# swacisko/ALGA

Hardware: AMD Instinct MI355X
Metric: overlap_edges_per_sec (higher is better)
Workload: dtype u32; 1 GPU; cfg4_50M_150bp: 50000000 x 150 bp reads, genome 250000000, seed 11, err 0.00 -> 90621096 nodes (both strands, duplicates removed), min_overlap 82, rsoemo 116; generated on the device (alga_amd.workload.device_build) in 1.0 s; nodes=90621096, edges=92350115

## Files before the change

alga_amd/csrc/engine.hip:

```cpp
#include <hip/hip_runtime.h>

#include <algorithm>
#include <chrono>
#include <cstdio>
#include <cstdlib>
#include <cstring>
#include <new>
#include <string>
#include <thread>
#include <vector>

#include "engine_internal.h"
#include "prefsuf_shard.h"

using namespace alga;

namespace {

using Prepared = AlgaPrepared;

int prepare(alga_engine *e, const alga_nodes *nodes, const alga_prefsuf_params *p, hipStream_t s, Prepared &out) {
    if (!nodes || !p) return alga_fail(e, ALGA_ERR_INVALID_ARGUMENT, "nodes/params must not be NULL");
    if (nodes->n < 0) return alga_fail(e, ALGA_ERR_INVALID_ARGUMENT, "negative node count");
    if (nodes->n > 0 && (!nodes->words || !nodes->len)) return alga_fail(e, ALGA_ERR_INVALID_ARGUMENT, "words/len must not be NULL");
// ... 5 lines not shown
    if (p->keys_shared < 0 || p->keys_shared > 2) return alga_fail(e, ALGA_ERR_INVALID_ARGUMENT, "keys_shared must be 0, 1 or 2");
    int rc;
    if ((rc = alga_ensure(e, e->counters, (CNT_TOTAL + 2) * sizeof(unsigned long long)))) return rc;
    HIP_TRY(e, hipMemsetAsync(e->counters.p, 0, (CNT_TOTAL + 2) * sizeof(unsigned long long), s));
    NodesDev nd;
    nd.words = nodes->words; nd.len = nodes->len; nd.from = nodes->align_from; nd.to = nodes->align_to;
    nd.n = nodes->n; nd.stride = nodes->stride_words;
    unsigned long long *cnt = (unsigned long long *) e->counters.p;
    int *d_maxlen = (int *) (cnt + CNT_TOTAL);
    unsigned long long mask_asym = 0;
    int min_len = 0;
    if (p->keys_shared == 2 && e->store_n == nodes->n && e->store_words == (const void *) nodes->words && e->stat_len == (const void *) nodes->len &&
        e->stat_from == (const void *) nodes->align_from && e->stat_to == (const void *) nodes->align_to) {
        out.max_len = e->stat_max_len; out.live = e->stat_live; mask_asym = e->stat_mask_asym; min_len = e->stat_min_len;
    } else {
        launch_node_stats(nd, cnt, d_maxlen, s);
        if ((rc = alga_check_launch(e, "k_node_stats"))) return rc;
        HIP_TRY(e, hipMemcpyAsync(e->h_counters, e->counters.p, (CNT_TOTAL + 2) * sizeof(unsigned long long), hipMemcpyDeviceToHost, s));
        HIP_TRY(e, hipStreamSynchronize(s));
        out.max_len = (int) (e->h_counters[CNT_TOTAL] & 0xFFFFFFFFull);
        min_len = out.max_len > 0 ? 0x7FFFFFFF - (int) (e->h_counters[CNT_TOTAL] >> 32) : 0;
        out.live = e->h_counters[CNT_LIVE_NODES];
        mask_asym = e->h_counters[CNT_MASK_ASYM];
        e->stat_max_len = out.max_len; e->stat_min_len = min_len; e->stat_live = out.live; e->stat_mask_asym = mask_asym;
        e->stat_len = (const void *) nodes->len; e->stat_from = (const void *) nodes->align_from; e->stat_to = (const void *) nodes->align_to;
    }
    out.nd = nd;
    out.uniform_len = (out.max_len > 0 && min_len == out.max_len && !nodes->align_from) ? out.max_len : 0;
    if ((int64_t) blocks_of(out.max_len) > (int64_t) nodes->stride_words)
        return alga_fail(e, ALGA_ERR_INVALID_ARGUMENT, "stride_words is smaller than the longest read needs");
    if (out.max_len > OL_MAX_NODE_LEN) return alga_fail(e, ALGA_ERR_CAPACITY, "a node is longer than 4 194 303 nt (overlap records keep the offset in 22 bits)");
// ... 107 lines not shown
        if ((rc = cluster_alloc(e, pp))) return rc;
        if (pp.keys_shared == 2) {
            const bool store_left = e->store_n == nd.n && e->store_words == (const void *) nd.words && e->store_eq == pp.cluster_eq && e->store_buckets == cc.n_buckets;
            const bool piles_serve = pile && e->pile_kept_pure && e->store_buckets == cc.n_buckets && e->store_eq == pp.cluster_eq;
            if (!(store_left || piles_serve) || src_begin < e->store_run_begin || src_end > e->store_run_end)
                return alga_fail(e, ALGA_ERR_INVALID_ARGUMENT, "keys_shared = 2: no entry array of this node set that covers the sources is left from the previous build");
            keys_only = pile && e->pile_keys_only;
        } else {
            int32_t run_begin = 0, run_end = nd.n;
            if (pp.keys_shared == 1) {
                if (e->keyed_n != nd.n || e->keyed_words != (const void *) nd.words || src_begin < e->keyed_begin || src_end > e->keyed_end)
                    return alga_fail(e, ALGA_ERR_INVALID_ARGUMENT, "keys_shared: alga_prefsuf_keys_device has not been called on this node set for a range that covers the sources");
                run_begin = e->keyed_begin; run_end = e->keyed_end;
            } else {
                keys_only = pile && e->opt_pile_runs != 0 && !e->expect_pairwise && !e->opt_pile_check;
                launch_cluster_keys(nd, cfg, cc, 0, nd.n, (uint32_t *) e->cl_keys[0].p, need_vals ? (uint32_t *) e->cl_vals[0].p : nullptr, (uint32_t *) e->cl_meta.p, e->cl_runs.p,
                                    (uint8_t *) e->cl_nruns.p, s, !keys_only);
                if ((rc = alga_check_launch(e, "k_node_runs"))) return rc;
            }
            HIP_TRY(e, hipEventRecord(e->ev[EV_KEYS], s));
            e->keyed_n = -1;
            e->store_n = -1;
            HIP_TRY(e, launch_cluster_sort(nd, cc, (uint32_t *) e->cl_keys[0].p, (uint32_t *) e->cl_vals[0].p, (uint32_t *) e->cl_keys[1].p,
                                           (uint32_t *) e->cl_vals[1].p, e->sort_temp.p, cluster_sort_temp_bytes((uint64_t) nd.n), pp.keys_shared == 1 || !need_vals,
                                           e->ev[EV_SORT], e->opt_test_unsorted_index != 0, s, e->opt_own_sort != 0));
            const bool dir_late = pile && e->opt_pile_dir >= 1;
            e->dir_late = dir_late;
            if (!dir_late) {
                HIP_TRY(e, launch_cluster_dir(nd, cc, (const uint32_t *) e->cl_keys[1].p, e->cl_dir.p, cnt + CNT_TOTAL + 1, nullptr, s));
                HIP_TRY(e, hipEventRecord(e->ev[EV_DIR], s));
            }
            e->pile_n = -1;
            if (pile) {
                rc = e->opt_test_pile_oom ? alga_fail(e, ALGA_ERR_OUT_OF_MEMORY, "pile_alloc (option test_pile_oom)") : pile_alloc(e, (uint64_t) nd.n, cc.n_buckets, s);
                if (rc == ALGA_ERR_OUT_OF_MEMORY) {
                    (void) hipGetLastError();
                    alga_release(e->cl_pile_tab); alga_release(e->cl_pile_rec); alga_release(e->cl_pile_rec2); alga_release(e->cl_pile_succ); alga_release(e->cl_pile_own);
                    alga_release(e->cl_pile_list);
                    e->pile_epoch = 0; e->pile_n = -1;
                    e->err.clear();
                    pile = false;
                    rc = ALGA_OK;
                    if (keys_only) {
                        launch_cluster_keys(nd, cfg, cc, 0, nd.n, (uint32_t *) e->cl_keys[0].p, (uint32_t *) e->cl_vals[0].p, (uint32_t *) e->cl_meta.p, e->cl_runs.p,
                                            (uint8_t *) e->cl_nruns.p, s, true);
                        if ((rc = alga_check_launch(e, "k_node_runs"))) return rc;
                        keys_only = false;
                    }
                } else if (rc) return rc;
            }
            if (pile) {
                launch_pile_sample(nd, cc, pp.uniform_len, (const uint32_t *) e->cl_keys[1].p, (const uint32_t *) e->cl_vals[1].p, e->cl_dir.p,
                                   (unsigned long long *) e->cl_pile_cnt.p, e->opt_pile >= 2 ? e->opt_pile - 1 : 0, s, e->opt_pile_dir >= 1);
                if ((rc = alga_check_launch(e, "k_pile_build<sample>"))) return rc;
            }
            e->pile_tab_index = pile && e->opt_pile_dir >= 2 && e->opt_pile_skip_gather && !cfg.stats;
            if (dir_late) {
                HIP_TRY(e, hipEventRecord(e->ev[EV_SAMPLE], s));
                HIP_TRY(e, launch_cluster_dir(nd, cc, (const uint32_t *) e->cl_keys[1].p, e->cl_dir.p, cnt + CNT_TOTAL + 1,
                                              e->pile_tab_index ? (const unsigned long long *) e->cl_pile_cnt.p : nullptr, s));
                HIP_TRY(e, hipEventRecord(e->ev[EV_DIR], s));
            }
            HIP_TRY(e, launch_cluster_gather(nd, cc, pp.cluster_eq, (const uint32_t *) e->cl_keys[1].p, (const uint32_t *) e->cl_vals[1].p, (const uint32_t *) e->cl_meta.p,
                                             pp.uniform_len, e->cl_store.p, (pile && e->opt_pile_skip_gather) ? (const unsigned long long *) e->cl_pile_cnt.p : nullptr, s));
            HIP_TRY(e, hipEventRecord(e->ev[EV_GATHER], s));
            if (pile) {
                if (e->pile_epoch >= 511u) {
                    HIP_TRY(e, hipMemsetAsync(e->cl_pile_tab.p, 0, e->cl_pile_tab.cap, s));
                    e->pile_epoch = 0;
                }
                e->pile_epoch++;
                const bool from_consensus = e->opt_pile_runs != 0;
                launch_pile_build(nd, cfg, cc, pp.uniform_len, (const uint32_t *) e->cl_keys[1].p, (const uint32_t *) e->cl_vals[1].p, e->cl_dir.p, e->cl_pile_rec.p, e->cl_pile_rec2.p, e->cl_pile_tab.p,
                                  e->pile_epoch, e->cl_pile_succ.p, e->cl_runs.p, pp.uniform_len - cfg.Lmin + 1, (const unsigned long long *) e->cl_pile_cnt.p,
                                  from_consensus ? (uint32_t *) e->cl_pile_own.p : nullptr, (from_consensus && e->opt_pile_runs_list) ? e->cl_pile_list.p : nullptr, s,
// ... 1175 lines not shown
```

alga_amd/csrc/prefsuf_cluster.hip:

```cpp
#include <hip/hip_runtime.h>
#include <algorithm>
#include "prefsuf_common.h"
#include "prefsuf_kernels.h"
#include "prefsuf_device.h"
#include "prefsuf_cluster_device.h"

namespace alga {


template <int TKW, bool WIDE, bool RUNS>
__global__ void __launch_bounds__(TK_ROWS) k_node_runs(NodesDev nd, PrefSufCfg cfg, ClusterCfg cc, int node_begin, int node_end,
                                                        uint32_t *__restrict__ keys, uint32_t *__restrict__ vals, uint32_t *__restrict__ meta,
                                                        uint2 *__restrict__ runs, uint8_t *__restrict__ nruns, const int32_t *__restrict__ id_list, const unsigned long long *__restrict__ id_count,
                                                        const unsigned long long *__restrict__ only_if_declined ) {
    if (only_if_declined && !pile_cnt_declines(only_if_declined)) return;
    __shared__ uint32_t s[TK_ROWS][TKW];
    __shared__ uint32_t stk[RUNS ? 2 * (NR_STACK + 1) : 1][TK_ROWS];
    __shared__ uint16_t rbuf[RUNS ? CL_RMAX + 1 : 1][TK_ROWS];
    const int list_n = id_list ? (int) min((unsigned long long) (node_end - node_begin), *id_count) : 0;
    __shared__ int sid[TK_ROWS];
    for (int blk = (int) blockIdx.x; id_list ? blk * TK_ROWS < list_n : node_begin + blk * TK_ROWS < node_end; blk += (int) gridDim.x) {
    const int base = node_begin + blk * TK_ROWS;
    const int nrows = id_list ? min(TK_ROWS, list_n - blk * TK_ROWS) : min(TK_ROWS, node_end - base);
    if (blk != (int) blockIdx.x) __syncthreads();
    if (id_list) {
// ... 66 lines not shown
            const uint32_t pk = order_key0(kmer_hash(funnel(x0, x1, r) & cc.lo_mask, funnel(x1, x2, r) & cc.hi_mask), e);
            cur0 = pk < cur0 ? pk : cur0;
        }
    }
    uint32_t key = 0xFFFFFFFFu, m = act ? (((uint32_t) len << 8) | (is_src ? CL_META_FROM : 0u)) : 0u;
    if (is_tgt) {
        uint32_t pmin = cur0;
        if (pmin == 0xFFFFFFFFu) {
            for (int k = 0; k < w; k++) { uint32_t h, pk; kmer_key(row, k, true, cc, h, pk); pmin = pk < pmin ? pk : pmin; }
        }
        uint32_t h, pk;
        kmer_key(row, (int) (pmin & 255u), true, cc, h, pk);
        key = tgt_sort_key(cluster_key(h, fs), pmin & 255u, fs);
        m = (pmin & 255u) | ((uint32_t) len << 8) | (is_src ? CL_META_FROM : 0u);
    }
    if (in) { keys[i] = key; if (vals) vals[i] = (uint32_t) i; meta[i] = m; }
    }
}

template <int EQ, bool UNIFORM>
__global__ void __launch_bounds__(256) k_tgt_gather(NodesDev nd, uint64_t count ,
                                                     const uint32_t *__restrict__ keys, const uint32_t *__restrict__ vals,
                                                     const uint32_t *__restrict__ meta, uint32_t uniform_meta, int fs, uint4 *__restrict__ store,
                                                     const unsigned long long *__restrict__ pile_cnt ) {
    if (pile_cnt && pile_cnt[1] * PILE_IRREGULAR_ONE_IN <= pile_cnt[0]) return;
    for (uint64_t t = (uint64_t) blockIdx.x * blockDim.x + threadIdx.x; t < count * EQ; t += (uint64_t) gridDim.x * blockDim.x) {
    const uint64_t j = t / EQ;
    const int c = (int) (t % EQ);
    const uint32_t key = keys[j];
    const uint32_t id = vals[j];
    const uint32_t *row = nd.words + (size_t) id * nd.stride;
// ... 8 lines not shown
        if (!UNIFORM) v.w = meta[id];
        else if (key != 0xFFFFFFFFu) v.w = uniform_meta | ((key >> fs) & ((1u << CL_MBITS) - 1u));
        else v.w = (uint32_t) nd.len[id] == (uniform_meta >> 8 & 0xFFFu) ? uniform_meta : 0u;
    }
    store[j * EQ + c] = v;
    }
}

constexpr int TD_TILE = 256, TD_HALO = 96;
__global__ void __launch_bounds__(TD_TILE) k_tgt_dir(const uint32_t *__restrict__ keys, uint64_t n, int shift, uint32_t n_buckets ,
                                                     uint32_t bucket_base , uint4 *__restrict__ dir,
                                                     unsigned long long *__restrict__ bad ,
                                                     const unsigned long long *__restrict__ pile_cnt ) {
    if (pile_cnt && pile_cnt_pure(pile_cnt)) return;
    __shared__ uint32_t sb[TD_TILE + TD_HALO + 1];
    const uint64_t base = (uint64_t) blockIdx.x * TD_TILE;
    const uint32_t nb3 = n_buckets << 3;
    auto tagged = [&](uint64_t k) -> uint32_t { if (k >= n) return nb3; const uint32_t x = keys[k]; return x == 0xFFFFFFFFu ? nb3 : (x >> (shift - 3)) - (bucket_base << 3); };
    for (int k = (int) threadIdx.x; k <= TD_TILE + TD_HALO; k += TD_TILE)
        sb[k] = (base == 0 && k == 0) ? 0xFFFFFFFFu : tagged(base + (uint64_t) k - 1u);
    __syncthreads();
    const int t = (int) threadIdx.x, lane = lane_id();
    const uint64_t j = base + (uint64_t) t;
    auto put = [&](int64_t b, const uint4 &rec) { dir[b] = rec; };
    auto tally = [](unsigned long long acc, uint32_t cls) { return acc + (0x0101010101010100ull << (8u * cls)); };
    if (j >= 1 && j < n && sb[t + 1] < sb[t]) atomicOr(bad, 1ull);
    const uint32_t b = sb[t + 1] >> 3;
    const bool start = j <= n && b != (sb[t] >> 3);
    if (start && b == n_buckets) put(b, make_uint4((uint32_t) j, 0u, 0u, 0u));
    const bool real = start && b != n_buckets;
    constexpr int TD_SHORT = 4;
    const bool is_short = real && (sb[t + 1 + TD_SHORT] >> 3) != b;
    if (is_short) {
// ... 47 lines not shown
            if (past) {
                for (; k < j0 + 256u; k++) {
                    const uint32_t x = tagged(k);
                    if ((x >> 3) != bb) break;
                    acc = tally(acc, x & 7u);
                }
                if (k >= j0 + 256u && (tagged(k) >> 3) == bb) {
                    uint64_t a = k, z = n;
                    while (z - a > 1) { const uint64_t mid = a + (z - a) / 2; if ((tagged(mid) >> 3) == bb) a = mid; else z = mid; }
                    k = z;
                }
            }
            const uint32_t c = (uint32_t) (k - j0);
            put(bb, make_uint4((uint32_t) j0, c, c <= 255u ? (uint32_t) acc : 0u, c <= 255u ? (uint32_t) (acc >> 32) : 0u));
        }
    }
}

#ifndef CL_OCC
#define CL_OCC 6
#endif

struct ByIdEntries {
    const uint32_t *skeys, *sids;
    uint32_t uniform_meta;
    const unsigned long long *pile_cnt;
    BucketIndex bx;
};
__device__ __forceinline__ void by_id_pair(const ByIdEntries &by, size_t ei, uint32_t n_nodes, uint32_t &key, uint32_t &id) {
    key = by.skeys[ei];
// ... 812 lines not shown
    c->idx_shift = 32 - bits;
    *eq = e;
    return true;
}

size_t cluster_sort_temp_bytes(uint64_t n) { return sort_u32_pairs_temp_bytes(n); }

void launch_cluster_keys(const NodesDev &nd, const PrefSufCfg &cfg, const ClusterCfg &cc, int32_t node_begin, int32_t node_end, uint32_t *keys, uint32_t *vals,
                         uint32_t *meta, void *runs, uint8_t *nruns, hipStream_t s, bool with_runs, const unsigned long long *only_if_declined) {
    if (node_end <= node_begin) return;
    const uint64_t m = (uint64_t) (node_end - node_begin);
    const unsigned long long *gate = only_if_declined;
    const dim3 grid((unsigned) (gate ? std::min<uint64_t>((m + TK_ROWS - 1) / TK_ROWS, 8192) : (m + TK_ROWS - 1) / TK_ROWS)), block(TK_ROWS);
    const int32_t *nol = nullptr; const unsigned long long *noc = nullptr;
#define NR_LAUNCH(TKW, WIDE) do { if (with_runs) hipLaunchKernelGGL((k_node_runs<TKW, WIDE, true>), grid, block, 0, s, nd, cfg, cc, (int) node_begin, (int) node_end, keys, vals, meta, (uint2 *) runs, nruns, nol, noc, gate); \
                                  else hipLaunchKernelGGL((k_node_runs<TKW, WIDE, false>), grid, block, 0, s, nd, cfg, cc, (int) node_begin, (int) node_end, keys, vals, meta, (uint2 *) runs, nruns, nol, noc, gate); } while (0)
    if (blocks_of(cfg.Lcap - 1) > 13 || (cfg.Lcap - 1) - cfg.Lmin + 1 > 64) NR_LAUNCH(21, true);
    else if (blocks_of(cfg.Lcap - 1) <= 9) NR_LAUNCH(11, false);
    else NR_LAUNCH(17, false);
#undef NR_LAUNCH
}

void launch_cluster_runs_list(const NodesDev &nd, const PrefSufCfg &cfg, const ClusterCfg &cc, const int32_t *ids, const unsigned long long *count, uint32_t cap, uint32_t grid_blocks,
                              void *runs, uint8_t *nruns, hipStream_t s) {
    if (cap == 0 || nd.n <= 0) return;
    const dim3 grid(std::max<uint32_t>(1u, std::min<uint32_t>(grid_blocks, (cap + TK_ROWS - 1) / TK_ROWS))), block(TK_ROWS);
    uint32_t *nok = nullptr;
#define NR_LAUNCH(TKW, WIDE) hipLaunchKernelGGL((k_node_runs<TKW, WIDE, true>), grid, block, 0, s, nd, cfg, cc, 0, (int) cap, nok, nok, nok, (uint2 *) runs, nruns, ids, count, (const unsigned long long *) nullptr)
    if (blocks_of(cfg.Lcap - 1) > 13 || (cfg.Lcap - 1) - cfg.Lmin + 1 > 64) NR_LAUNCH(21, true);
    else if (blocks_of(cfg.Lcap - 1) <= 9) NR_LAUNCH(11, false);
    else NR_LAUNCH(17, false);
#undef NR_LAUNCH
}

__global__ void __launch_bounds__(256) k_iota(uint32_t *__restrict__ v, uint32_t n) {
    for (uint32_t i = blockIdx.x * 256u + threadIdx.x; i < n; i += gridDim.x * 256u) v[i] = i;
}

hipError_t launch_cluster_store(const NodesDev &nd, const ClusterCfg &cc, uint32_t *keys, uint32_t *vals, uint32_t *keys2, uint32_t *vals2,
                                void *sort_temp, size_t sort_temp_bytes, void *dir, bool fill_vals,
                                hipEvent_t ev_sorted, unsigned long long *bad_flag, bool test_skip_sort, hipStream_t s, bool own_sort) {
    const hipError_t err = launch_cluster_sort(nd, cc, keys, vals, keys2, vals2, sort_temp, sort_temp_bytes, fill_vals, ev_sorted, test_skip_sort, s, own_sort);
    return err != hipSuccess ? err : launch_cluster_dir(nd, cc, keys2, dir, bad_flag, nullptr, s);
}

hipError_t launch_cluster_sort(const NodesDev &nd, const ClusterCfg &cc, uint32_t *keys, uint32_t *vals, uint32_t *keys2, uint32_t *vals2, void *sort_temp, size_t sort_temp_bytes,
                               bool fill_vals, hipEvent_t ev_sorted, bool test_skip_sort, hipStream_t s, bool own_sort) {
    if (nd.n <= 0) return hipSuccess;
    const uint64_t n = (uint64_t) nd.n;
    if (fill_vals && (!own_sort || test_skip_sort)) hipLaunchKernelGGL(k_iota, dim3((unsigned) std::min<uint64_t>((n + 255) / 256, 8192)), dim3(256), 0, s, vals, (uint32_t) n);
    hipError_t err = hipSuccess;
    if (test_skip_sort) {
        err = hipMemcpyAsync(keys2, keys, n * sizeof(uint32_t), hipMemcpyDeviceToDevice, s);
        if (err == hipSuccess) err = hipMemcpyAsync(vals2, vals, n * sizeof(uint32_t), hipMemcpyDeviceToDevice, s);
    } else err = sort_u32_pairs(sort_temp, sort_temp_bytes, keys, keys2, own_sort ? (const uint32_t *) nullptr : vals, vals2, n, cc.idx_shift - 3, s, own_sort);
    if (err != hipSuccess) return err;
    if (ev_sorted) (void) hipEventRecord(ev_sorted, s);
    return hipSuccess;
// ... 1 lines not shown

constexpr int DF_UNROLL = 4;
__global__ void __launch_bounds__(256) k_dir_fill(uint4 *__restrict__ dir, uint64_t n_rec, const unsigned long long *__restrict__ pile_cnt) {
    if (pile_cnt && pile_cnt_pure(pile_cnt)) return;
    const uint4 z = make_uint4(0u, 0u, 0u, 0u);
    for (uint64_t p = (uint64_t) blockIdx.x * (256u * DF_UNROLL); p < n_rec; p += (uint64_t) gridDim.x * (256u * DF_UNROLL)) {
#pragma unroll
        for (int u = 0; u < DF_UNROLL; u++) {
            const uint64_t i = p + (uint64_t) u * 256u + threadIdx.x;
            if (i < n_rec) dir[i] = z;
        }
    }
}

hipError_t launch_cluster_dir(const NodesDev &nd, const ClusterCfg &cc, const uint32_t *keys2, void *dir, unsigned long long *bad_flag, const unsigned long long *only_if_no_pure_piles,
                              hipStream_t s) {
    if (nd.n <= 0) return hipSuccess;
    const uint64_t n = (uint64_t) nd.n, n_rec = (uint64_t) cc.n_buckets + 2;
    if (only_if_no_pure_piles)
        hipLaunchKernelGGL(k_dir_fill, dim3((unsigned) std::min<uint64_t>((n_rec + 256 * DF_UNROLL - 1) / (256 * DF_UNROLL), 1u << 17)), dim3(256), 0, s, (uint4 *) dir, n_rec,
                           only_if_no_pure_piles);
    else {
        const hipError_t err = hipMemsetAsync(dir, 0, n_rec * 16, s);
        if (err != hipSuccess) return err;
    }
    hipLaunchKernelGGL(k_tgt_dir, dim3((unsigned) ((n + 1 + TD_TILE - 1) / TD_TILE)), dim3(TD_TILE), 0, s, keys2, n, cc.idx_shift, cc.n_buckets, 0u, (uint4 *) dir, bad_flag, only_if_no_pure_piles);
    return hipGetLastError();
}

hipError_t launch_cluster_gather(const NodesDev &nd, const ClusterCfg &cc, int eq, const uint32_t *keys2, const uint32_t *vals2, const uint32_t *meta, int uniform_len,
                                 void *store, const unsigned long long *pile_cnt, hipStream_t s) {
    if (nd.n <= 0) return hipSuccess;
    const uint64_t n = (uint64_t) nd.n;
    const uint64_t pieces = n * (uint64_t) eq;
    const unsigned g = (unsigned) std::min<uint64_t>((pieces + 255) / 256, 1u << 16);
    const int fs = cc.idx_shift - CL_MBITS;
    const uint32_t um = uniform_len > 0 ? (((uint32_t) uniform_len << 8) | CL_META_FROM) : 0u;
#define TG_LAUNCH(E, U) hipLaunchKernelGGL((k_tgt_gather<E, U>), dim3(g), dim3(256), 0, s, nd, n, keys2, vals2, meta, um, fs, (uint4 *) store, pile_cnt)
#define TG_EQ(E) do { if (uniform_len > 0) TG_LAUNCH(E, true); else TG_LAUNCH(E, false); } while (0)
    if (eq == 2)      TG_EQ(2);
    else if (eq == 3) TG_EQ(3);
// ... 138 lines not shown
```

alga_amd/csrc/prefsuf_kernels.h:

```cpp
#pragma once
#include <hip/hip_runtime.h>
#include <stddef.h>
#include <stdint.h>
#include "prefsuf_common.h"

namespace alga {

struct alga_edge_dev { int32_t src, dst, offset; };

void launch_restride(const uint32_t *in, int stride_in, uint32_t *out, int stride_out, uint64_t n, hipStream_t s);
void launch_widen_len(const void *in, int elem_bytes , int32_t *out, uint64_t n, hipStream_t s);
void launch_compact_edges(const alga_edge_dev *edges, int32_t n, uint64_t n_edges, uint8_t *deg, uint32_t *dst, uint8_t *off, unsigned long long *bad, hipStream_t s);
void launch_expand_twins(const uint32_t *in, int stride_in, const int32_t *len , uint32_t *out, int stride_out, uint64_t n_pairs, hipStream_t s);
void launch_node_stats(const NodesDev &nd, unsigned long long *counters, int *max_len , hipStream_t s);

uint32_t seed_buckets_for(uint64_t live_nodes, int fill_x10);
uint32_t seed_filter_bits_for(uint64_t live_nodes);
void launch_seed_build(const NodesDev &nd, const PrefSufCfg &cfg, unsigned long long *table, uint32_t n_buckets, uint32_t *filter,
                       uint32_t filter_bits, hipStream_t s);

struct ProbeBig { int32_t *list; uint32_t list_cap; uint32_t count; void *items; uint32_t item_cap; };
int    local_item_capacity();
int    local_big_limit();
size_t probe_big_bytes(int n_cu, uint32_t count, int local, uint32_t item_cap);

void launch_probe(const NodesDev &nd, const PrefSufCfg &cfg, const unsigned long long *table, uint32_t n_buckets,
                  const uint32_t *filter, uint32_t filter_bits, int32_t src_begin, int32_t src_end, uint32_t *rec_dst, unsigned long long *rec_val, uint64_t rec_cap,
                  unsigned long long *counters, int n_cu, int local , uint32_t *deg , unsigned long long *first ,
                  const ProbeBig *big , hipStream_t s);
// ... 5 lines not shown

bool       cluster_plan(const PrefSufCfg &cfg, int max_len, uint64_t live, int bucket_log2_bias, ClusterCfg *c, int *eq);
size_t     cluster_sort_temp_bytes(uint64_t n);
void       launch_cluster_keys(const NodesDev &nd, const PrefSufCfg &cfg, const ClusterCfg &cc, int32_t node_begin, int32_t node_end, uint32_t *keys,
                               uint32_t *vals, uint32_t *meta, void *runs, uint8_t *nruns, hipStream_t s, bool with_runs = true ,
                               const unsigned long long *only_if_declined = nullptr );
void       launch_cluster_runs_list(const NodesDev &nd, const PrefSufCfg &cfg, const ClusterCfg &cc, const int32_t *ids, const unsigned long long *count, uint32_t cap,
                                    uint32_t grid_blocks, void *runs, uint8_t *nruns, hipStream_t s);
hipError_t launch_cluster_store(const NodesDev &nd, const ClusterCfg &cc, uint32_t *keys, uint32_t *vals, uint32_t *keys2 , uint32_t *vals2, void *sort_temp,
                                size_t sort_temp_bytes, void *dir, bool fill_vals, hipEvent_t ev_sorted ,
                                unsigned long long *bad_flag ,
                                bool test_skip_sort , hipStream_t s, bool own_sort = true);
hipError_t launch_cluster_sort(const NodesDev &nd, const ClusterCfg &cc, uint32_t *keys, uint32_t *vals, uint32_t *keys2, uint32_t *vals2, void *sort_temp, size_t sort_temp_bytes,
                               bool fill_vals, hipEvent_t ev_sorted, bool test_skip_sort, hipStream_t s, bool own_sort = true);
hipError_t launch_cluster_dir(const NodesDev &nd, const ClusterCfg &cc, const uint32_t *keys2, void *dir, unsigned long long *bad_flag, const unsigned long long *only_if_no_pure_piles,
                              hipStream_t s);
hipError_t launch_cluster_gather(const NodesDev &nd, const ClusterCfg &cc, int eq, const uint32_t *keys2, const uint32_t *vals2, const uint32_t *meta,
                                 int uniform_len , void *store,
                                 const unsigned long long *pile_cnt , hipStream_t s);
uint64_t   cluster_record_slack(int n_cu, uint64_t n_src);
void       launch_probe_clustered(const NodesDev &nd, const PrefSufCfg &cfg, const ClusterCfg &cc, int eq, const void *store, const void *dir,
                                  const void *runs, const uint8_t *nruns, int32_t src_begin, int32_t src_end, const int32_t *src_list, int32_t src_base, uint32_t *rec_dst, unsigned long long *rec_val, uint64_t rec_cap,
                                  unsigned long long *counters, int n_cu, uint32_t *deg, unsigned long long *first, const ProbeBig *big,
                                  const unsigned long long *list_count ,
                                  int sw , hipStream_t s,
                                  const uint32_t *skeys = nullptr, const uint32_t *sids = nullptr, int uniform_len = 0,
                                  const unsigned long long *pile_cnt = nullptr ,
                                  const void *tab = nullptr , uint32_t epoch = 0);
void       launch_probe_stream(const NodesDev &nd, const PrefSufCfg &cfg, const ClusterCfg &cc, int eq, const void *store, const void *dir,
                               const void *runs, const uint8_t *nruns, int32_t src_begin, int32_t src_end, bool by_key ,
                               unsigned long long *counters, int n_cu, uint32_t *deg, unsigned long long *first, unsigned long long *second, int32_t *defer_list,
// ... 90 lines not shown
```

alga_amd/csrc/prefsuf_kernels.hip:

```cpp
#include <hip/hip_runtime.h>
#include <algorithm>
#include "prefsuf_common.h"
#include "prefsuf_kernels.h"
#include "prefsuf_device.h"
#include "prefsuf_cluster_device.h"

namespace alga {

__global__ void __launch_bounds__(256) k_node_stats(NodesDev nd, unsigned long long *counters, int *max_len) {
    __shared__ int s_max[4], s_min[4];
    __shared__ unsigned long long s_live[4];
    int m = 0, mn = 0x7FFFFFFF;
    unsigned long long live = 0, asym = 0;
    auto one = [&](int l, int64_t i) {
        m = l > m ? l : m;
        mn = (l > 0 && l < mn) ? l : mn;
        live += l > 0;
        if (nd.to && l > 0 && !nd.to[i] && (nd.from == nullptr || nd.from[i])) asym++;
    };
    const int64_t gid = (int64_t) blockIdx.x * blockDim.x + threadIdx.x, gsz = (int64_t) gridDim.x * blockDim.x;
    int64_t done = 0;
    if ((reinterpret_cast<uintptr_t>(nd.len) & 15u) == 0) {
        const int64_t nq = (int64_t) nd.n >> 2;
        const int4 *len4 = reinterpret_cast<const int4 *>(nd.len);
        for (int64_t q = gid; q < nq; q += gsz) { const int4 l = len4[q]; one(l.x, 4 * q); one(l.y, 4 * q + 1); one(l.z, 4 * q + 2); one(l.w, 4 * q + 3); }
        done = 4 * nq;
    }
    for (int64_t i = done + gid; i < nd.n; i += gsz) one(nd.len[i], i);
#pragma unroll
    for (int o = 32; o > 0; o >>= 1) { int t = __shfl_xor(m, o); m = t > m ? t : m; t = __shfl_xor(mn, o); mn = t < mn ? t : mn; }
    live = wave_sum_u64(live);
    asym = wave_sum_u64(asym);
    const int wave = (int) (threadIdx.x >> 6);
    if (lane_id() == 0) { s_max[wave] = m; s_min[wave] = mn; s_live[wave] = live; if (asym) atomicAdd(&counters[CNT_MASK_ASYM], asym); }
    __syncthreads();
    if (threadIdx.x == 0) {
        for (int w = 1; w < 4; w++) { m = s_max[w] > m ? s_max[w] : m; mn = s_min[w] < mn ? s_min[w] : mn; live += s_live[w]; }
        if (m > 0) { atomicMax(max_len, m); atomicMax(max_len + 1, 0x7FFFFFFF - mn); }
        if (live) atomicAdd(&counters[CNT_LIVE_NODES], live);
    }
}

__device__ __forceinline__ uint32_t seed_bucket(uint64_t h, uint32_t n_buckets) { return __umulhi((uint32_t) h, n_buckets); }
__device__ __forceinline__ uint32_t seed_taglen(uint64_t h, int len) {
    return ((uint32_t) (h >> 41) << 9) | (uint32_t) (len > 511 ? 511 : len);
}

__device__ __forceinline__ uint32_t seed_filter_index(uint64_t h, uint32_t filter_mask) { return (uint32_t) (h >> 32) & filter_mask; }

__global__ void __launch_bounds__(256) k_seed_build(NodesDev nd, PrefSufCfg cfg, unsigned long long *table, uint32_t n_buckets,
                                                     uint32_t *filter, uint32_t filter_mask) {
    int i = blockIdx.x * blockDim.x + threadIdx.x;
    if (i >= nd.n) return;
    int len = nd.len[i];
// ... 920 lines not shown
            if (piled && (v[k].x == 0u || v[k].y == 0u)) a = f2[g];
            if (piled && (v[k].z == 0u || v[k].w == 0u)) b = f2[g + 1];
            s += source_degree(v[k].x, piled, a.x) + source_degree(v[k].y, piled, a.y) + source_degree(v[k].z, piled, b.x) + source_degree(v[k].w, piled, b.y);
        }
    } else {
        for (int k = 0; k < SCAN_ITEMS; k++) {
            const uint64_t i = base + (uint64_t) k * SCAN_BLOCK + threadIdx.x;
            if (i < n) { const uint32_t dg = deg[i]; s += source_degree(dg, piled, (piled && dg == 0u) ? first[i] : LOCAL_FIRST_NONE); }
        }
    }
    uint32_t tot;
    block_exclusive_scan(s, &tot, lds);
    if (threadIdx.x == 0) tile_sums[blockIdx.x] = tot;
}

__global__ void __launch_bounds__(1024) k_scan_spine_serial(uint64_t *tile_sums, uint32_t n_tiles) {
    __shared__ uint64_t lds[16];
    const int lane = lane_id(), wave = (int) (threadIdx.x >> 6);
    const uint64_t per = ((uint64_t) n_tiles + 1023u) / 1024u;
    const uint64_t beg = min((uint64_t) threadIdx.x * per, (uint64_t) n_tiles), end = min(beg + per, (uint64_t) n_tiles);
    uint64_t sum = 0;
    for (uint64_t i = beg; i < end; i++) sum += tile_sums[i];
    uint64_t inc = sum;
#pragma unroll
    for (int o = 1; o < 64; o <<= 1) {
        const uint32_t lo = (uint32_t) __shfl_up((int) (uint32_t) inc, o), hi = (uint32_t) __shfl_up((int) (uint32_t) (inc >> 32), o);
        if (lane >= o) inc += ((uint64_t) hi << 32) | lo;
    }
    if (lane == 63) lds[wave] = inc;
    __syncthreads();
    uint64_t run = inc - sum;
    for (int w = 0; w < wave; w++) run += lds[w];
    for (uint64_t i = beg; i < end; i++) { const uint64_t v = tile_sums[i]; tile_sums[i] = run; run += v; }
    if (threadIdx.x == 1023) tile_sums[n_tiles] = run;
}

__global__ void __launch_bounds__(SCAN_BLOCK) k_emit_scan_tiles(int32_t src_base, uint64_t n, const uint32_t *__restrict__ deg, const unsigned long long *__restrict__ first,
                                                                 const unsigned long long *__restrict__ second, const unsigned long long *__restrict__ pile_cnt,
                                                                 const uint64_t *__restrict__ tile_sums, uint32_t *__restrict__ out, alga_edge_dev *__restrict__ edges,
                                                                 uint32_t slot_stride) {
    __shared__ uint32_t lds[8];
    const bool piled = pile_cnt != nullptr && !pile_cnt_declines(pile_cnt);
    const int lane = lane_id(), wave = (int) (threadIdx.x >> 6);
    const uint64_t wbase = (uint64_t) blockIdx.x * SCAN_TILE + (uint64_t) wave * (64 * SCAN_ITEMS) + (uint64_t) lane;
    uint32_t d[SCAN_ITEMS];
    unsigned long long f[SCAN_ITEMS];
#pragma unroll
    for (int k = 0; k < SCAN_ITEMS; k++) { const uint64_t i = wbase + 64u * k; d[k] = i < n ? deg[i] : 0u; }
#pragma unroll
// ... 137 lines not shown
    if (n_edges == 0) return;
    hipLaunchKernelGGL(k_compact_edges, dim3((unsigned) std::min<uint64_t>((n_edges + 255) / 256, 1u << 16)), dim3(256), 0, s, edges, n, n_edges, deg, dst, off, bad);
}

void launch_expand_twins(const uint32_t *in, int stride_in, const int32_t *len, uint32_t *out, int stride_out, uint64_t n_pairs, hipStream_t s) {
    if (n_pairs == 0) return;
    hipLaunchKernelGGL(k_expand_twins, dim3((unsigned) std::min<uint64_t>((n_pairs * (uint64_t) stride_out + 255) / 256, 1u << 16)), dim3(256), 0, s, in, stride_in, len, out,
                       stride_out, n_pairs);
}

void launch_restride(const uint32_t *in, int stride_in, uint32_t *out, int stride_out, uint64_t n, hipStream_t s) {
    if (n == 0) return;
    hipLaunchKernelGGL(k_restride, dim3((unsigned) std::min<uint64_t>((n * (uint64_t) stride_out + 255) / 256, 1u << 16)), dim3(256), 0, s, in, stride_in, out, stride_out, n);
}

void launch_node_stats(const NodesDev &nd, unsigned long long *counters, int *max_len, hipStream_t s) {
    if (nd.n <= 0) return;
    unsigned g = std::min<unsigned>(grid_for((uint64_t) nd.n, 256), 1024u);
    hipLaunchKernelGGL(k_node_stats, dim3(g), dim3(256), 0, s, nd, counters, max_len);
}

uint32_t seed_buckets_for(uint64_t live, int fill_x10) {
    if (fill_x10 < 5) fill_x10 = 5;
    if (fill_x10 > 60) fill_x10 = 60;
    uint64_t nb = (live * 10 + (uint64_t) fill_x10 - 1) / (uint64_t) fill_x10;
    if (nb < 64) nb = 64;
    return (uint32_t) std::min<uint64_t>(nb, 0x7FFFFFFFull);
}

uint32_t seed_filter_bits_for(uint64_t live) {
    const uint64_t want = live * 8;
    uint64_t bits = 1ull << 16;
    while (bits < want) bits <<= 1;
    if (bits <= (1ull << 25)) return (uint32_t) bits;
// ... 201 lines not shown
```

Measured before the change: 5.485 billion edges/s.

## Retune node stats, directory, key and spine-scan kernels for grid and throughput

Several unrelated kernel-level changes. k_node_stats now uses 1024-thread blocks with unrolled int4 loads, an alignment head, a CU-sized grid, and a single block-level atomic for the asymmetry counter. k_tgt_dir becomes grid-strided and is capped to a chip-sized grid when piles may skip it. k_node_runs skips writing meta when only keys are needed and lengths are uniform. The serial spine scan is rewritten as a chunked, LDS-staged, coalesced block scan with prefetch. These target launch overhead, uncoalesced serial memory access and redundant stores, at the risk of lower parallelism in the capped grids.

After: 5.518 billion edges/s (median of 6 runs). Within noise of the previous version (+0.6%).

```diff
diff --git a/alga_amd/csrc/engine.hip b/alga_amd/csrc/engine.hip
--- a/alga_amd/csrc/engine.hip
+++ b/alga_amd/csrc/engine.hip
@@ -43,7 +43,7 @@
         e->stat_from == (const void *) nodes->align_from && e->stat_to == (const void *) nodes->align_to) {
         out.max_len = e->stat_max_len; out.live = e->stat_live; mask_asym = e->stat_mask_asym; min_len = e->stat_min_len;
     } else {
-        launch_node_stats(nd, cnt, d_maxlen, s);
+        launch_node_stats(nd, cnt, d_maxlen, e->n_cu, s);
         if ((rc = alga_check_launch(e, "k_node_stats"))) return rc;
         HIP_TRY(e, hipMemcpyAsync(e->h_counters, e->counters.p, (CNT_TOTAL + 2) * sizeof(unsigned long long), hipMemcpyDeviceToHost, s));
         HIP_TRY(e, hipStreamSynchronize(s));
@@ -181,8 +181,8 @@
                 run_begin = e->keyed_begin; run_end = e->keyed_end;
             } else {
                 keys_only = pile && e->opt_pile_runs != 0 && !e->expect_pairwise && !e->opt_pile_check;
-                launch_cluster_keys(nd, cfg, cc, 0, nd.n, (uint32_t *) e->cl_keys[0].p, need_vals ? (uint32_t *) e->cl_vals[0].p : nullptr, (uint32_t *) e->cl_meta.p, e->cl_runs.p,
-                                    (uint8_t *) e->cl_nruns.p, s, !keys_only);
+                launch_cluster_keys(nd, cfg, cc, 0, nd.n, (uint32_t *) e->cl_keys[0].p, need_vals ? (uint32_t *) e->cl_vals[0].p : nullptr,
+                                    (keys_only && pp.uniform_len > 0) ? nullptr : (uint32_t *) e->cl_meta.p, e->cl_runs.p, (uint8_t *) e->cl_nruns.p, s, !keys_only);
                 if ((rc = alga_check_launch(e, "k_node_runs"))) return rc;
             }
             HIP_TRY(e, hipEventRecord(e->ev[EV_KEYS], s));
@@ -194,7 +194,7 @@
             const bool dir_late = pile && e->opt_pile_dir >= 1;
             e->dir_late = dir_late;
             if (!dir_late) {
-                HIP_TRY(e, launch_cluster_dir(nd, cc, (const uint32_t *) e->cl_keys[1].p, e->cl_dir.p, cnt + CNT_TOTAL + 1, nullptr, s));
+                HIP_TRY(e, launch_cluster_dir(nd, cc, (const uint32_t *) e->cl_keys[1].p, e->cl_dir.p, cnt + CNT_TOTAL + 1, nullptr, e->n_cu, s));
                 HIP_TRY(e, hipEventRecord(e->ev[EV_DIR], s));
             }
             e->pile_n = -1;
@@ -225,7 +225,7 @@
             if (dir_late) {
                 HIP_TRY(e, hipEventRecord(e->ev[EV_SAMPLE], s));
                 HIP_TRY(e, launch_cluster_dir(nd, cc, (const uint32_t *) e->cl_keys[1].p, e->cl_dir.p, cnt + CNT_TOTAL + 1,
-                                              e->pile_tab_index ? (const unsigned long long *) e->cl_pile_cnt.p : nullptr, s));
+                                              e->pile_tab_index ? (const unsigned long long *) e->cl_pile_cnt.p : nullptr, e->n_cu, s));
                 HIP_TRY(e, hipEventRecord(e->ev[EV_DIR], s));
             }
             HIP_TRY(e, launch_cluster_gather(nd, cc, pp.cluster_eq, (const uint32_t *) e->cl_keys[1].p, (const uint32_t *) e->cl_vals[1].p, (const uint32_t *) e->cl_meta.p,
diff --git a/alga_amd/csrc/prefsuf_cluster.hip b/alga_amd/csrc/prefsuf_cluster.hip
--- a/alga_amd/csrc/prefsuf_cluster.hip
+++ b/alga_amd/csrc/prefsuf_cluster.hip
@@ -8,7 +8,7 @@
 namespace alga {
 
 
-template <int TKW, bool WIDE, bool RUNS>
+template <int TKW, bool WIDE, bool RUNS, bool META = true>
 __global__ void __launch_bounds__(TK_ROWS) k_node_runs(NodesDev nd, PrefSufCfg cfg, ClusterCfg cc, int node_begin, int node_end,
                                                         uint32_t *__restrict__ keys, uint32_t *__restrict__ vals, uint32_t *__restrict__ meta,
                                                         uint2 *__restrict__ runs, uint8_t *__restrict__ nruns, const int32_t *__restrict__ id_list, const unsigned long long *__restrict__ id_count,
@@ -105,7 +105,7 @@
         key = tgt_sort_key(cluster_key(h, fs), pmin & 255u, fs);
         m = (pmin & 255u) | ((uint32_t) len << 8) | (is_src ? CL_META_FROM : 0u);
     }
-    if (in) { keys[i] = key; if (vals) vals[i] = (uint32_t) i; meta[i] = m; }
+    if (in) { keys[i] = key; if (vals) vals[i] = (uint32_t) i; if (META) meta[i] = m; }
     }
 }
 
@@ -144,9 +144,12 @@
                                                      const unsigned long long *__restrict__ pile_cnt ) {
     if (pile_cnt && pile_cnt_pure(pile_cnt)) return;
     __shared__ uint32_t sb[TD_TILE + TD_HALO + 1];
-    const uint64_t base = (uint64_t) blockIdx.x * TD_TILE;
     const uint32_t nb3 = n_buckets << 3;
     auto tagged = [&](uint64_t k) -> uint32_t { if (k >= n) return nb3; const uint32_t x = keys[k]; return x == 0xFFFFFFFFu ? nb3 : (x >> (shift - 3)) - (bucket_base << 3); };
+    const uint64_t n_tiles = (n + 1 + TD_TILE - 1) / TD_TILE;
+    for (uint64_t tile = blockIdx.x; tile < n_tiles; tile += gridDim.x) {
+    const uint64_t base = tile * TD_TILE;
+    if (tile != blockIdx.x) __syncthreads();
     for (int k = (int) threadIdx.x; k <= TD_TILE + TD_HALO; k += TD_TILE)
         sb[k] = (base == 0 && k == 0) ? 0xFFFFFFFFu : tagged(base + (uint64_t) k - 1u);
     __syncthreads();
@@ -224,6 +227,7 @@
             const uint32_t c = (uint32_t) (k - j0);
             put(bb, make_uint4((uint32_t) j0, c, c <= 255u ? (uint32_t) acc : 0u, c <= 255u ? (uint32_t) (acc >> 32) : 0u));
         }
+    }
     }
 }
 
@@ -1066,7 +1070,8 @@
     const dim3 grid((unsigned) (gate ? std::min<uint64_t>((m + TK_ROWS - 1) / TK_ROWS, 8192) : (m + TK_ROWS - 1) / TK_ROWS)), block(TK_ROWS);
     const int32_t *nol = nullptr; const unsigned long long *noc = nullptr;
 #define NR_LAUNCH(TKW, WIDE) do { if (with_runs) hipLaunchKernelGGL((k_node_runs<TKW, WIDE, true>), grid, block, 0, s, nd, cfg, cc, (int) node_begin, (int) node_end, keys, vals, meta, (uint2 *) runs, nruns, nol, noc, gate); \
-                                  else hipLaunchKernelGGL((k_node_runs<TKW, WIDE, false>), grid, block, 0, s, nd, cfg, cc, (int) node_begin, (int) node_end, keys, vals, meta, (uint2 *) runs, nruns, nol, noc, gate); } while (0)
+                                  else if (meta) hipLaunchKernelGGL((k_node_runs<TKW, WIDE, false>), grid, block, 0, s, nd, cfg, cc, (int) node_begin, (int) node_end, keys, vals, meta, (uint2 *) runs, nruns, nol, noc, gate); \
+                                  else hipLaunchKernelGGL((k_node_runs<TKW, WIDE, false, false>), grid, block, 0, s, nd, cfg, cc, (int) node_begin, (int) node_end, keys, vals, meta, (uint2 *) runs, nruns, nol, noc, gate); } while (0)
     if (blocks_of(cfg.Lcap - 1) > 13 || (cfg.Lcap - 1) - cfg.Lmin + 1 > 64) NR_LAUNCH(21, true);
     else if (blocks_of(cfg.Lcap - 1) <= 9) NR_LAUNCH(11, false);
     else NR_LAUNCH(17, false);
@@ -1093,7 +1098,7 @@
                                 void *sort_temp, size_t sort_temp_bytes, void *dir, bool fill_vals,
                                 hipEvent_t ev_sorted, unsigned long long *bad_flag, bool test_skip_sort, hipStream_t s, bool own_sort) {
     const hipError_t err = launch_cluster_sort(nd, cc, keys, vals, keys2, vals2, sort_temp, sort_temp_bytes, fill_vals, ev_sorted, test_skip_sort, s, own_sort);
-    return err != hipSuccess ? err : launch_cluster_dir(nd, cc, keys2, dir, bad_flag, nullptr, s);
+    return err != hipSuccess ? err : launch_cluster_dir(nd, cc, keys2, dir, bad_flag, nullptr, 0 , s);
 }
 
 hipError_t launch_cluster_sort(const NodesDev &nd, const ClusterCfg &cc, uint32_t *keys, uint32_t *vals, uint32_t *keys2, uint32_t *vals2, void *sort_temp, size_t sort_temp_bytes,
@@ -1125,17 +1130,20 @@
 }
 
 hipError_t launch_cluster_dir(const NodesDev &nd, const ClusterCfg &cc, const uint32_t *keys2, void *dir, unsigned long long *bad_flag, const unsigned long long *only_if_no_pure_piles,
-                              hipStream_t s) {
+                              int n_cu, hipStream_t s) {
     if (nd.n <= 0) return hipSuccess;
     const uint64_t n = (uint64_t) nd.n, n_rec = (uint64_t) cc.n_buckets + 2;
+    const uint64_t chip = (uint64_t) std::max(1, n_cu) * 64u;
     if (only_if_no_pure_piles)
-        hipLaunchKernelGGL(k_dir_fill, dim3((unsigned) std::min<uint64_t>((n_rec + 256 * DF_UNROLL - 1) / (256 * DF_UNROLL), 1u << 17)), dim3(256), 0, s, (uint4 *) dir, n_rec,
+        hipLaunchKernelGGL(k_dir_fill, dim3((unsigned) std::min<uint64_t>((n_rec + 256 * DF_UNROLL - 1) / (256 * DF_UNROLL), chip)), dim3(256), 0, s, (uint4 *) dir, n_rec,
                            only_if_no_pure_piles);
     else {
         const hipError_t err = hipMemsetAsync(dir, 0, n_rec * 16, s);
         if (err != hipSuccess) return err;
     }
-    hipLaunchKernelGGL(k_tgt_dir, dim3((unsigned) ((n + 1 + TD_TILE - 1) / TD_TILE)), dim3(TD_TILE), 0, s, keys2, n, cc.idx_shift, cc.n_buckets, 0u, (uint4 *) dir, bad_flag, only_if_no_pure_piles);
+    const uint64_t tiles = (n + 1 + TD_TILE - 1) / TD_TILE;
+    hipLaunchKernelGGL(k_tgt_dir, dim3((unsigned) (only_if_no_pure_piles ? std::min<uint64_t>(tiles, chip) : tiles)), dim3(TD_TILE), 0, s, keys2, n, cc.idx_shift, cc.n_buckets, 0u, (uint4 *) dir,
+                       bad_flag, only_if_no_pure_piles);
     return hipGetLastError();
 }
 
diff --git a/alga_amd/csrc/prefsuf_kernels.h b/alga_amd/csrc/prefsuf_kernels.h
--- a/alga_amd/csrc/prefsuf_kernels.h
+++ b/alga_amd/csrc/prefsuf_kernels.h
@@ -12,7 +12,7 @@
 void launch_widen_len(const void *in, int elem_bytes , int32_t *out, uint64_t n, hipStream_t s);
 void launch_compact_edges(const alga_edge_dev *edges, int32_t n, uint64_t n_edges, uint8_t *deg, uint32_t *dst, uint8_t *off, unsigned long long *bad, hipStream_t s);
 void launch_expand_twins(const uint32_t *in, int stride_in, const int32_t *len , uint32_t *out, int stride_out, uint64_t n_pairs, hipStream_t s);
-void launch_node_stats(const NodesDev &nd, unsigned long long *counters, int *max_len , hipStream_t s);
+void launch_node_stats(const NodesDev &nd, unsigned long long *counters, int *max_len , int n_cu, hipStream_t s);
 
 uint32_t seed_buckets_for(uint64_t live_nodes, int fill_x10);
 uint32_t seed_filter_bits_for(uint64_t live_nodes);
@@ -48,7 +48,7 @@
 hipError_t launch_cluster_sort(const NodesDev &nd, const ClusterCfg &cc, uint32_t *keys, uint32_t *vals, uint32_t *keys2, uint32_t *vals2, void *sort_temp, size_t sort_temp_bytes,
                                bool fill_vals, hipEvent_t ev_sorted, bool test_skip_sort, hipStream_t s, bool own_sort = true);
 hipError_t launch_cluster_dir(const NodesDev &nd, const ClusterCfg &cc, const uint32_t *keys2, void *dir, unsigned long long *bad_flag, const unsigned long long *only_if_no_pure_piles,
-                              hipStream_t s);
+                              int n_cu , hipStream_t s);
 hipError_t launch_cluster_gather(const NodesDev &nd, const ClusterCfg &cc, int eq, const uint32_t *keys2, const uint32_t *vals2, const uint32_t *meta,
                                  int uniform_len , void *store,
                                  const unsigned long long *pile_cnt , hipStream_t s);
diff --git a/alga_amd/csrc/prefsuf_kernels.hip b/alga_amd/csrc/prefsuf_kernels.hip
--- a/alga_amd/csrc/prefsuf_kernels.hip
+++ b/alga_amd/csrc/prefsuf_kernels.hip
@@ -7,9 +7,10 @@
 
 namespace alga {
 
-__global__ void __launch_bounds__(256) k_node_stats(NodesDev nd, unsigned long long *counters, int *max_len) {
-    __shared__ int s_max[4], s_min[4];
-    __shared__ unsigned long long s_live[4];
+constexpr int NS_UNROLL = 4, NS_BLOCK = 1024;
+__global__ void __launch_bounds__(NS_BLOCK) k_node_stats(NodesDev nd, unsigned long long *counters, int *max_len) {
+    __shared__ int s_max[NS_BLOCK / 64], s_min[NS_BLOCK / 64];
+    __shared__ unsigned long long s_live[NS_BLOCK / 64], s_asym[NS_BLOCK / 64];
     int m = 0, mn = 0x7FFFFFFF;
     unsigned long long live = 0, asym = 0;
     auto one = [&](int l, int64_t i) {
@@ -18,26 +19,35 @@
         live += l > 0;
         if (nd.to && l > 0 && !nd.to[i] && (nd.from == nullptr || nd.from[i])) asym++;
     };
+    auto four = [&](const int4 &l, int64_t i) { one(l.x, i); one(l.y, i + 1); one(l.z, i + 2); one(l.w, i + 3); };
     const int64_t gid = (int64_t) blockIdx.x * blockDim.x + threadIdx.x, gsz = (int64_t) gridDim.x * blockDim.x;
-    int64_t done = 0;
-    if ((reinterpret_cast<uintptr_t>(nd.len) & 15u) == 0) {
-        const int64_t nq = (int64_t) nd.n >> 2;
-        const int4 *len4 = reinterpret_cast<const int4 *>(nd.len);
-        for (int64_t q = gid; q < nq; q += gsz) { const int4 l = len4[q]; one(l.x, 4 * q); one(l.y, 4 * q + 1); one(l.z, 4 * q + 2); one(l.w, 4 * q + 3); }
-        done = 4 * nq;
-    }
-    for (int64_t i = done + gid; i < nd.n; i += gsz) one(nd.len[i], i);
+    const uintptr_t addr = reinterpret_cast<uintptr_t>(nd.len);
+    const int64_t to16 = (int64_t) (((16u - (uint32_t) (addr & 15u)) & 15u) >> 2);
+    const int64_t head = ((addr & 3u) || to16 > (int64_t) nd.n) ? (int64_t) nd.n : to16;
+    const int64_t nq = ((int64_t) nd.n - head) >> 2;
+    const int4 *len4 = reinterpret_cast<const int4 *>(nd.len + head);
+    constexpr int64_t PIECE = (int64_t) NS_BLOCK * NS_UNROLL;
+    for (int64_t p = (int64_t) blockIdx.x * PIECE; p < nq; p += (int64_t) gridDim.x * PIECE) {
+        int4 l[NS_UNROLL];
+#pragma unroll
+        for (int u = 0; u < NS_UNROLL; u++) { const int64_t q = p + u * NS_BLOCK + threadIdx.x; l[u] = q < nq ? len4[q] : make_int4(0, 0, 0, 0); }
+#pragma unroll
+        for (int u = 0; u < NS_UNROLL; u++) { const int64_t q = p + u * NS_BLOCK + threadIdx.x; if (q < nq) four(l[u], head + 4 * q); }
+    }
+    for (int64_t i = gid; i < head; i += gsz) one(nd.len[i], i);
+    for (int64_t i = head + 4 * nq + gid; i < nd.n; i += gsz) one(nd.len[i], i);
 #pragma unroll
     for (int o = 32; o > 0; o >>= 1) { int t = __shfl_xor(m, o); m = t > m ? t : m; t = __shfl_xor(mn, o); mn = t < mn ? t : mn; }
     live = wave_sum_u64(live);
     asym = wave_sum_u64(asym);
     const int wave = (int) (threadIdx.x >> 6);
-    if (lane_id() == 0) { s_max[wave] = m; s_min[wave] = mn; s_live[wave] = live; if (asym) atomicAdd(&counters[CNT_MASK_ASYM], asym); }
+    if (lane_id() == 0) { s_max[wave] = m; s_min[wave] = mn; s_live[wave] = live; s_asym[wave] = asym; }
     __syncthreads();
     if (threadIdx.x == 0) {
-        for (int w = 1; w < 4; w++) { m = s_max[w] > m ? s_max[w] : m; mn = s_min[w] < mn ? s_min[w] : mn; live += s_live[w]; }
+        for (int w = 1; w < NS_BLOCK / 64; w++) { m = s_max[w] > m ? s_max[w] : m; mn = s_min[w] < mn ? s_min[w] : mn; live += s_live[w]; asym += s_asym[w]; }
         if (m > 0) { atomicMax(max_len, m); atomicMax(max_len + 1, 0x7FFFFFFF - mn); }
         if (live) atomicAdd(&counters[CNT_LIVE_NODES], live);
+        if (asym) atomicAdd(&counters[CNT_MASK_ASYM], asym);
     }
 }
 
@@ -988,25 +998,42 @@
     if (threadIdx.x == 0) tile_sums[blockIdx.x] = tot;
 }
 
+constexpr int SPINE_ITEMS = 4, SPINE_CHUNK = 1024 * SPINE_ITEMS;
 __global__ void __launch_bounds__(1024) k_scan_spine_serial(uint64_t *tile_sums, uint32_t n_tiles) {
-    __shared__ uint64_t lds[16];
-    const int lane = lane_id(), wave = (int) (threadIdx.x >> 6);
-    const uint64_t per = ((uint64_t) n_tiles + 1023u) / 1024u;
-    const uint64_t beg = min((uint64_t) threadIdx.x * per, (uint64_t) n_tiles), end = min(beg + per, (uint64_t) n_tiles);
-    uint64_t sum = 0;
-    for (uint64_t i = beg; i < end; i++) sum += tile_sums[i];
-    uint64_t inc = sum;
-#pragma unroll
-    for (int o = 1; o < 64; o <<= 1) {
-        const uint32_t lo = (uint32_t) __shfl_up((int) (uint32_t) inc, o), hi = (uint32_t) __shfl_up((int) (uint32_t) (inc >> 32), o);
-        if (lane >= o) inc += ((uint64_t) hi << 32) | lo;
-    }
-    if (lane == 63) lds[wave] = inc;
-    __syncthreads();
-    uint64_t run = inc - sum;
-    for (int w = 0; w < wave; w++) run += lds[w];
-    for (uint64_t i = beg; i < end; i++) { const uint64_t v = tile_sums[i]; tile_sums[i] = run; run += v; }
-    if (threadIdx.x == 1023) tile_sums[n_tiles] = run;
+    __shared__ uint64_t buf[SPINE_CHUNK];
+    __shared__ uint64_t wtot[16];
+    const int t = (int) threadIdx.x, lane = lane_id(), wave = t >> 6;
+    uint64_t carry = 0;
+    uint64_t nxt[SPINE_ITEMS];
+#pragma unroll
+    for (int k = 0; k < SPINE_ITEMS; k++) { const uint64_t i = (uint64_t) (k * 1024 + t); nxt[k] = i < n_tiles ? tile_sums[i] : 0ull; }
+    for (uint64_t base = 0; base < n_tiles; base += SPINE_CHUNK) {
+#pragma unroll
+        for (int k = 0; k < SPINE_ITEMS; k++) buf[k * 1024 + t] = nxt[k];
+#pragma unroll
+        for (int k = 0; k < SPINE_ITEMS; k++) { const uint64_t i = base + SPINE_CHUNK + (uint64_t) (k * 1024 + t); nxt[k] = i < n_tiles ? tile_sums[i] : 0ull; }
+        __syncthreads();
+        uint64_t v[SPINE_ITEMS], sum = 0;
+#pragma unroll
+        for (int k = 0; k < SPINE_ITEMS; k++) { v[k] = buf[t * SPINE_ITEMS + k]; sum += v[k]; }
+        uint64_t inc = sum;
+#pragma unroll
+        for (int o = 1; o < 64; o <<= 1) {
+            const uint32_t lo = (uint32_t) __shfl_up((int) (uint32_t) inc, o), hi = (uint32_t) __shfl_up((int) (uint32_t) (inc >> 32), o);
+            if (lane >= o) inc += ((uint64_t) hi << 32) | lo;
+        }
+        if (lane == 63) wtot[wave] = inc;
+        __syncthreads();
+        uint64_t run = carry + inc - sum;
+#pragma unroll
+        for (int w = 0; w < 16; w++) { const uint64_t x = wtot[w]; run += w < wave ? x : 0ull; carry += x; }
+#pragma unroll
+        for (int k = 0; k < SPINE_ITEMS; k++) { buf[t * SPINE_ITEMS + k] = run; run += v[k]; }
+        __syncthreads();
+#pragma unroll
+        for (int k = 0; k < SPINE_ITEMS; k++) { const uint64_t i = base + (uint64_t) (k * 1024 + t); if (i < n_tiles) tile_sums[i] = buf[k * 1024 + t]; }
+    }
+    if (t == 0) tile_sums[n_tiles] = carry;
 }
 
 __global__ void __launch_bounds__(SCAN_BLOCK) k_emit_scan_tiles(int32_t src_base, uint64_t n, const uint32_t *__restrict__ deg, const unsigned long long *__restrict__ first,
@@ -1174,10 +1201,10 @@
     hipLaunchKernelGGL(k_restride, dim3((unsigned) std::min<uint64_t>((n * (uint64_t) stride_out + 255) / 256, 1u << 16)), dim3(256), 0, s, in, stride_in, out, stride_out, n);
 }
 
-void launch_node_stats(const NodesDev &nd, unsigned long long *counters, int *max_len, hipStream_t s) {
+void launch_node_stats(const NodesDev &nd, unsigned long long *counters, int *max_len, int n_cu, hipStream_t s) {
     if (nd.n <= 0) return;
-    unsigned g = std::min<unsigned>(grid_for((uint64_t) nd.n, 256), 1024u);
-    hipLaunchKernelGGL(k_node_stats, dim3(g), dim3(256), 0, s, nd, counters, max_len);
+    unsigned g = std::min<unsigned>(grid_for((uint64_t) nd.n, NS_BLOCK * 4 * NS_UNROLL), (unsigned) std::max(1, n_cu) * 2u);
+    hipLaunchKernelGGL(k_node_stats, dim3(g), dim3(NS_BLOCK), 0, s, nd, counters, max_len);
 }
 
 uint32_t seed_buckets_for(uint64_t live, int fill_x10) {
```
